# open-speech/HTK

Hardware: AMD Instinct MI355X
Metric: herest_gmm_frame_state_loglik_per_sec (higher is better)
Workload: dtype f32 (scores: bf16x3 split operands, fp32 accumulate) + f64 (alpha / beta with fp32-transcendental log-add, accumulators); 1 GPU; HERest EM iteration (pass + accumulator all-reduce + model update), 5000 tied states x 16 mix, D=39, 1250 x 500-frame utterances per GPU (BASELINE config[2]: 10k utterances sharded 8-way); states=5000, mix=16, utts_per_gpu=1250, frames=500, chunks=1, update=HERest -m 3 -v 0.01, on the device

## Files before the change

### htk_amd/capi.py

```python
from __future__ import annotations

import ctypes as C
import os

import numpy as np

from . import abi

HERE = os.path.dirname(os.path.abspath(__file__))
LIBPATH = os.path.join(HERE, "libhtk_amd.so")

LZERO = -1.0e10
LSMALL = -0.5e10
NOPRUNE = 1.0e20
UPMEANS, UPVARS, UPTRANS, UPMIXES = 1, 2, 4, 8
UPALL = 15
UPMAP = 32
UTT_OK, UTT_SKIPPED, UTT_ETEE, UTT_EALPHA = 1, 0, -7332, -7390


def _stream(s):
    return s if s is None or isinstance(s, C.c_void_p) else int(s)


# ... 275 lines not shown
    def pack_ranges(self, ranges, wire: int, dst_ptr: int, stream=None):
        self._ranges(lib().htkamd_accs_pack_ranges, ranges, wire, dst_ptr, stream)

    def unpack_ranges(self, ranges, wire: int, src_ptr: int, stream=None):
        self._ranges(lib().htkamd_accs_unpack_ranges, ranges, wire, src_ptr, stream)

    def split(self, v: np.ndarray) -> dict:
        m, L = self.model, self.lay
        GD = m.G * m.D
        return dict(vec=v, mu=v[L.mu:L.mu + GD].reshape(m.G, m.D), muOcc=v[L.muOcc:L.muOcc + m.G],
                    va=v[L.va:L.va + GD].reshape(m.G, m.D), vaOcc=v[L.vaOcc:L.vaOcc + m.G],
                    wt=v[L.wt:L.wt + m.C], wtOcc=v[L.wtOcc:L.tr], tr=v[L.tr:L.trOcc], trOcc=v[L.trOcc:L.nEgs],
                    nEgs=v[L.nEgs:L.nEgs + m.H], totalPr=v[L.totalPr], totalT=v[L.totalT], nUttDone=v[L.nUttDone],
                    nUttSkipped=v[L.nUttSkipped], nEval=v[L.nEval])


def fb_config(pruneInit=NOPRUNE, pruneInc=0.0, pruneLim=NOPRUNE, minFrwdP=10.0, uFlags=UPALL, scoreMode=0):
    return FbConfig(pruneInit, pruneInc, pruneLim, minFrwdP, uFlags, scoreMode)


class ForwardBackward(_Handle):
    _destroy = "htkamd_fb_destroy"

    def __init__(self, model: Model, debug: bool = False, force_general: bool = False, no_state_path: bool = False, stats_list: str = "auto", no_lr_path: bool = False):
        self.model = model
        self.h = C.c_void_p()
        check(lib().htkamd_fb_create(model.h, C.byref(self.h)), "fb_create")
        flags = (1 if debug else 0) | (2 if force_general else 0) | (4 if no_state_path else 0) | {"auto": 0, "tiny": 8, "off": 16}[stats_list] | (32 if no_lr_path else 0)
        if flags:
            check(lib().htkamd_fb_set_debug(self.h, flags), "fb_set_debug")
        self.nUtt = 0
        self._keep = None

    def prepare(self, dX_ptr: int, frameOff: np.ndarray, labOff: np.ndarray, labs: np.ndarray, stream=None):
        frameOff = np.ascontiguousarray(frameOff, np.int32); labOff = np.ascontiguousarray(labOff, np.int32)
        labs = np.ascontiguousarray(labs, np.int32)
        self.nUtt = len(frameOff) - 1
        self._keep = (frameOff, labOff, labs)
        b = BatchDesc(self.nUtt, dX_ptr, _p(frameOff), _p(labOff), _p(labs))
        check(lib().htkamd_fb_prepare(self.h, C.byref(b), _stream(stream)), "fb_prepare")

    def execute(self, cfg: FbConfig, accs: Accs, stream=None):
        check(lib().htkamd_fb_execute(self.h, C.byref(cfg), accs.h, _stream(stream)), "fb_execute")

    def execute_begin(self, cfg: FbConfig, accs: Accs, stream=None) -> bool:
        d = C.c_int(0)
        check(lib().htkamd_fb_execute_begin(self.h, C.byref(cfg), accs.h, _stream(stream), C.byref(d)), "fb_execute_begin")
        return bool(d.value)

    def execute_mix(self, state0: int, state1: int, stream=None):
        check(lib().htkamd_fb_execute_mix(self.h, state0, state1, _stream(stream)), "fb_execute_mix")
# ... 9 lines not shown
    def prepared_current(self) -> bool:
        return bool(lib().htkamd_fb_prepared_current(self.h))

    def frame_states(self) -> int:
        return int(lib().htkamd_fb_frame_states(self.h))

    def kernel_times(self):
        t = (C.c_double * 4)()
        check(lib().htkamd_fb_kernel_times(self.h, t), "fb_kernel_times")
        return list(t)

    def set_event_mode(self, mode: int):
        check(lib().htkamd_fb_set_event_mode(self.h, mode), "fb_set_event_mode")

    def kernel_times5(self):
        t = (C.c_double * 5)()
        check(lib().htkamd_fb_kernel_times5(self.h, t), "fb_kernel_times5")
        return list(t)

    def mix_counts(self):
        t = (C.c_longlong * 2)()
        check(lib().htkamd_fb_mix_counts(self.h, t), "fb_mix_counts")
        return int(t[0]), int(t[1])

    def score_work(self):
        t = (C.c_longlong * 3)()
        check(lib().htkamd_fb_score_work(self.h, t), "fb_score_work")
        return int(t[0]), int(t[1]), int(t[2])

    def trellis(self, u: int, want_alpha: bool = True):
        T = C.c_int(); Q = C.c_int(); mN = C.c_int()
        check(lib().htkamd_fb_get_trellis(self.h, u, None, None, None, None, None, None, None,
                                          C.byref(T), C.byref(Q), C.byref(mN), None), "fb_get_trellis")
        T, Q, mN = T.value, Q.value, mN.value
        d = dict(beta=np.empty((T, Q, mN)), alpha=np.empty((T, Q, mN)) if want_alpha else None,
                 outp=np.empty((T, Q, mN), np.float32), qLo=np.zeros(T, np.int32), qHi=np.zeros(T, np.int32),
                 aLo=np.zeros(T, np.int32), aHi=np.zeros(T, np.int32))
        check(lib().htkamd_fb_get_trellis(self.h, u, _p(d["beta"]), _p(d["alpha"]), _p(d["outp"]),
                                          _p(d["qLo"]), _p(d["qHi"]), _p(d["aLo"]), _p(d["aHi"]), None, None, None, None),
              "fb_get_trellis")
        return d


class Viterbi(_Handle):
    _destroy = "htkamd_viterbi_destroy"

# ... 1607 lines not shown
```

### htk_amd/csrc/fb.hip

```cpp
#include <hip/hip_runtime.h>
#include <cstdio>
#include <cstdlib>
#include <cstring>
#include <cmath>
#include <algorithm>
#include <vector>
#include <thread>
#include <mutex>
#include <condition_variable>
#include <functional>
#include "internal.h"
#include "hipcheck.h"
#include "kernels.h"
#include "devbuf.h"

static constexpr char fbOwner[] = "fb";
typedef DevBufT<fbOwner> DevBuf;

struct PrepPool {
   std::vector<std::thread> th;
   std::mutex mu;
   std::condition_variable cvGo, cvDone;
   std::function<void(int)> job;
   int generation = 0, pending = 0, nJobs = 0;
// ... 99 lines not shown
   Range general() const { return of(FB_LANE_PER_MODEL, 0); } int nGeneral() const { return general().n; }
   int nLr() const { return off[N] - of(FB_LEFT_TO_RIGHT, 1).first; }
   bool anyOffLr() const { return of(FB_LEFT_TO_RIGHT, 1).first > 0; }
private:
   int off[N + 1] = {};
};

struct ResLayout {
   size_t nUtt;
   size_t status() const { return sizeof(double) * nUtt; }
   size_t counter() const { return (sizeof(double) + sizeof(int)) * nUtt; }
   size_t flag() const { return counter() + sizeof(int); } size_t bytes() const { return counter() + 2 * sizeof(int); }
};

enum { UTT_NO_TEE = 1, UTT_ALL_LR = 2 };

struct htkamd_fb : BatchTables {
   htkamd_model *m = nullptr;
   int nUtt = 0;
   int debug = 0;
   int forceGeneral = 0;
   int noStatePath = 0;
   int noLrPath = 0;
   int topoVersion = 0;
   std::vector<unsigned char> uttFlags;
   UttClasses cls;
   size_t gamTotal = 0, betaWTotal = 0, alphaWTotal = 0;
   int totalFrames = 0, nCellsMax = 1, QMax = 1, TMax = 1, blockDim = 64;
   long long frameStates = 0;
   const float *dX = nullptr;
   DevBuf d_arena;
   DevBuf d_qLo, d_qHi, d_aLo, d_aHi, d_outp, d_beta, d_gam, d_alpha, d_pr;
   DevBuf d_betaW;
   DevBuf d_tmE, d_tmMaxP;
   DevBuf d_outpU;
   DevBuf d_alphaW, d_qBeam, d_aBeam, d_trPart, d_hits, d_hitCtl;
   DevBuf d_sink;
   DevBuf d_stCnt, d_stBucket;
   DevBuf d_laneRec;
   bool mixStateLast = false;
   bool mixDeferred = false;
   FbArgs *faMix = nullptr;
   const int *qBeamLast = nullptr;
   DevBuf d_transOff, d_trOccOff, d_counter;
   DevBuf d_rec, d_recSorted, d_recCtl;
   int recCapForce = 0;
   PrepPool *pool = nullptr; std::vector<PrepChunk> *chunks = nullptr;
   void *h_arena = nullptr; size_t h_arenaCap = 0;
   void *h_res = nullptr; size_t h_resCap = 0;
   hipEvent_t evRes = nullptr; bool resPending = false;
   bool f16Pass = false;
   hipEvent_t ev[6] = {}, evK[2] = {}, evCopy = nullptr;
   hipStream_t resStream = nullptr;
   bool timed = false, copyPending = false, scored = false;
   int evMode = 0, evModeLast = 0;
   ResLayout res() const { return {(size_t)nUtt}; }
};

static bool compat_revisit(const htkamd_model *m) { return (m->compat & HTKAMD_COMPAT_STREAM_REVISIT) && m->NSt > 1 && m->NSt != 3 && !m->tiedMix; }

extern "C" int htkamd_fb_create(htkamd_model *m, htkamd_fb **out)
{
// ... 16 lines not shown
   return HTKAMD_OK;
}

extern "C" void htkamd_fb_destroy(htkamd_fb *fb)
{
   if (!fb) return;
   if (fb->h_arena) (void)hipHostFree(fb->h_arena);
   if (fb->h_res) (void)hipHostFree(fb->h_res);
   delete fb->pool; delete fb->chunks; delete fb->faMix;
   for (hipEvent_t v : fb->ev) if (v) (void)hipEventDestroy(v);
   for (hipEvent_t v : {fb->evCopy, fb->evRes, fb->evK[0], fb->evK[1]}) if (v) (void)hipEventDestroy(v);
   if (fb->resStream) (void)hipStreamDestroy(fb->resStream);
   delete fb;
}

extern "C" int htkamd_fb_set_debug(htkamd_fb *fb, int on)
{
   if (!fb) { htkamd_set_error("fb_set_debug: NULL"); return HTKAMD_EINVAL; }
   fb->debug = on & 1;
   fb->forceGeneral = (on & 2) ? 1 : 0;
   fb->noStatePath = (on & 4) ? 1 : 0;
   fb->recCapForce = (on & 8) ? 128 : ((on & 16) ? -1 : 0);
   fb->noLrPath = (on & 32) ? 1 : 0;
   return HTKAMD_OK;
}

static int prep_utterance(htkamd_fb *fb, const htkamd_batch_desc *b, int u, PrepChunk &C)
{
   const htkamd_model *m = fb->m;
   std::vector<int> &evLo = C.evLo, &evHi = C.evHi;
      UttDesc &d = fb->utt[u];
      const int T = b->frameOff[u + 1] - b->frameOff[u], Q = b->labOff[u + 1] - b->labOff[u];
      const int *labs = b->labs + b->labOff[u];
      d.T = T; d.Q = Q; d.frame0 = b->frameOff[u];
      d.q0 = (int)C.mN.size(); d.cell0 = (int)C.cQ.size(); d.slot0 = (int)C.slotState.size();
      d.status = HTKAMD_UTT_OK; d.nEval = 0;
      d.outp0 = C.outp; d.beta0 = C.beta; d.gam0 = C.gam;
      unsigned char &flags = fb->uttFlags[u];
      flags = UTT_NO_TEE | UTT_ALL_LR;
      if (T <= 0 || Q <= 0) {
         for (int t = 0; t < T; t++) { fb->taperLo[d.frame0 + t] = 0; fb->taperHi[d.frame0 + t] = 0; fb->qBeamNP[d.frame0 + t] = 1; }
         d.status = HTKAMD_UTT_SKIPPED; d.nCells = d.nSlots = 0; d.thr0 = (int)C.thrCell.size(); d.nThr = 0; return HTKAMD_OK;
      }
      int nCells = 0, nSlots = 0, qt = 0, prevDm = 1;
      for (int q = 1; q <= Q; q++) {
         const int h = labs[q - 1];
// ... 404 lines not shown
}

static const int clsW[4] = {1, 2, 4, 8};

static int fb_reserve_lr(htkamd_fb *fb, const htkamd_fb_config *cfg, FbArgs &fa, bool fastLadd, hipStream_t s)
{
   const htkamd_model *m = fb->m;
   int rc;
   size_t rows = 0;
   for (int W : clsW) rows += (size_t)fb->cls.of(FB_LEFT_TO_RIGHT, W).n * htkamd_stats_lr_chunks(fb->TMax) * W;
   const size_t nfr = fb->totalFrames ? fb->totalFrames : 1;
   if ((rc = fb->d_laneRec.reserve(sizeof(LaneRec) * (fb->slotState.size() + 1))) || (rc = fb->d_sink.reserve(256))) return rc;
   fa.laneRec = (LaneRec *)fb->d_laneRec.p; fa.sink = (double *)fb->d_sink.p;
   if ((rc = fb->d_alphaW.reserve(sizeof(double) * (fb->alphaWTotal + 64))) || (rc = fb->d_qBeam.reserve(sizeof(int) * (nfr + 2))) ||
       (rc = fb->d_aBeam.reserve(sizeof(int) * (nfr + 2))) || (rc = fb->d_trPart.reserve(sizeof(double) * htkamd_stats_lr_row_doubles() * (rows + 256))) ||
       (rc = fb->d_hits.reserve(sizeof(MixHit) * (rows * htkamd_stats_lr_region_cap() + 64))) || (rc = fb->d_hitCtl.reserve(sizeof(int) * (rows + 1))))
      return rc;
   fa.alphaW = (double *)fb->d_alphaW.p; fa.qBeam = (int *)fb->d_qBeam.p; fa.aBeam = (int *)fb->d_aBeam.p; fa.trPart = (double *)fb->d_trPart.p;
   fa.hits = (MixHit *)fb->d_hits.p; fa.hitCtl = (int *)fb->d_hitCtl.p; fa.nHitRegions = (int)rows; fa.hitRegionCap = htkamd_stats_lr_region_cap();
   fa.hitSlots = (m->NSt > 1 || m->tiedMix) ? 1 : 0;
   fa.qBeamNP = fb->qBeamNP.dev;
   if (htkamd_beta_lr_is_lean(fa, fastLadd)) fa.qBeam = const_cast<int *>(fb->qBeamNP.dev);
   fb->qBeamLast = fa.qBeam;
   fb->mixStateLast = false;
   fa.fastMath = fastLadd ? 1 : 0;
   if (fb->recCapForce == 0 && !fa.hitSlots && m->maxM <= 16 && (m->D == 39 || m->D == 26 || m->D == 13) &&
       (cfg->uFlags & (HTKAMD_UPMEANS | HTKAMD_UPVARS | HTKAMD_UPMIXES))) {
      size_t cap = 64;
      while (cap < 65536 && cap * (size_t)m->S < (size_t)16 * fb->totalFrames) cap <<= 1;
      while (cap > 64 && cap * (size_t)m->S * sizeof(HitS) > ((size_t)1 << 30)) cap >>= 1;
      { const char *e = getenv("HTKAMD_ST_CAP"); if (e && atoi(e) > 0) cap = (size_t)atoi(e); }
      if ((rc = fb->d_stCnt.reserve(sizeof(int) * (3 * (size_t)m->S + 4))) || (rc = fb->d_stBucket.reserve(sizeof(HitS) * cap * (size_t)m->S))) return rc;
      fb->mixStateLast = true;
      fa.stCnt = (int *)fb->d_stCnt.p; fa.nTiedStates = m->S; fa.stBucket = (HitS *)fb->d_stBucket.p; fa.stCap = (int)cap;
      HIPCHECK(hipMemsetAsync(fa.stCnt, 0, sizeof(int) * (3 * (size_t)m->S + 4), s));
   }
   return HTKAMD_OK;
}

struct FamilyKernels { int family; int (*beta)(const FbArgs &, int, bool, hipStream_t); int (*alpha)(const FbArgs &, int, bool, hipStream_t); };
static const FamilyKernels familyKernels[] = {{FB_LANE_PER_MODEL, htkamd_launch_beta_w, htkamd_launch_alpha_w},
                                              {FB_LANE_PER_STATE, htkamd_launch_beta_s, htkamd_launch_alpha_s},
                                              {FB_LEFT_TO_RIGHT, htkamd_launch_beta_lr, htkamd_launch_alpha_lr}};

static int fb_recursions(htkamd_fb *fb, const FbArgs &fa, const LdsSizes &lds, bool fastLadd, bool noEv, hipStream_t s)
{
// ... 43 lines not shown
          (rc = fb->d_recCtl.reserve(sizeof(int) * (3 * ((size_t)m->G + 1) + 1 + (size_t)m->G / 2048 + 2))))
         return rc;
      fa.rec = (MixRec *)fb->d_rec.p; fa.recSorted = (MixRec *)fb->d_recSorted.p; fa.recCap = (int)cap; fa.G = m->G; fa.recCtl = (int *)fb->d_recCtl.p;
   }
   if (m->tiedMix || m->NSt > 1) {
      fa.stateCompOff = m->d_stateCompOff; fa.rec = nullptr;
      if (fb->nUtt > nLr && (rc = m->tiedMix ? htkamd_launch_mixstats_tm(fa, s) : htkamd_launch_mixstats_ms(fa, s))) return rc;
      if (nLr > 0 && (rc = htkamd_launch_mixhits_streams(fa, m->tiedMix != 0, s))) return rc;
      return HTKAMD_OK;
   }
   const bool dense = fb->nUtt > nLr && fa.gamTotal > 0, listed = nLr > 0;
   if ((rc = htkamd_launch_mixstats(fa, s, dense, listed, defer))) return rc;
   if (defer && listed && !dense && htkamd_mixstate_applies(fa)) {
      if (!fb->faMix) fb->faMix = new FbArgs();
      *fb->faMix = fa;
      fb->mixDeferred = true;
   }
   return HTKAMD_OK;
}

static int fb_execute_impl(htkamd_fb *fb, const htkamd_fb_config *cfg, htkamd_accs *accs, void *stream, bool defer)
{
   if (!fb || !cfg || !accs) { htkamd_set_error("fb_execute: NULL argument"); return HTKAMD_EINVAL; }
   fb->mixDeferred = false;
   if (accs->m != fb->m) { htkamd_set_error("fb_execute: accumulators belong to a different model"); return HTKAMD_EINVAL; }
   if (fb->nUtt == 0) return HTKAMD_OK;
   const htkamd_model *m = fb->m;
   hipStream_t s = (hipStream_t)stream;
   if (fb->topoVersion != m->topoVersion) {
      htkamd_set_error("fb_execute: the model's minimum durations changed since htkamd_fb_prepare (a re-estimated transition reached or left zero): prepare the batch again");
      return HTKAMD_EINVAL;
   }
   const ScoreArgs sa = fb_score_args(fb, cfg);
   if (cfg->scoreMode & ~(HTKAMD_SCORE_MFMA | HTKAMD_SCORE_FASTLADD | HTKAMD_SCORE_BF16 | HTKAMD_SCORE_F16 | HTKAMD_SCORE_SOUTP | HTKAMD_SCORE_DIAGC)) { htkamd_set_error("fb_execute: unknown score mode %d", cfg->scoreMode); return HTKAMD_EINVAL; }
   const bool fastLadd = (cfg->scoreMode & HTKAMD_SCORE_FASTLADD) != 0;
   FbArgs fa = fb_args(fb, cfg, accs);
   const LdsSizes lds = fb_lds_sizes(fa);

   int rc;
   if (fb->copyPending) HIPCHECK(hipStreamWaitEvent(s, fb->evCopy, 0));
   const bool noEv = fb->evMode == 1;
   HIPCHECK(hipEventRecord(fb->ev[0], s));
   if (m->tiedMix) {
      fa.tmE = (float *)fb->d_tmE.p; fa.tmMaxP = (float *)fb->d_tmMaxP.p; fa.tmPoolOff = m->d_tmPoolOff; fa.tmPool = m->tmPool; fa.totalFrames = fb->totalFrames;
      fa.tmTasks = fb->tasks.dev; fa.tmNTasks = (int)fb->tasks.size(); fa.tmSlotState = sa.slotState; fa.tmOut = sa.out;
      fa.compWeight = m->d_compWeight; fa.var = m->d_var;
      if ((rc = htkamd_launch_tm_score(fa, s))) return rc;
// ... 111 lines not shown
   if (!fb->timed) { htkamd_set_error("fb_kernel_times: nothing executed yet"); return HTKAMD_EINVAL; }
   HIPCHECK(hipEventSynchronize(fb->ev[5]));
   for (int i = 0; i < 5; i++) {
      float ms = 0.f;
      if (i == 0 && fb->scored) HIPCHECK(hipEventElapsedTime(&ms, fb->evK[0], fb->evK[1]));
      else if (fb->evModeLast == 1) { out[i] = -1.0; continue; }
      else HIPCHECK(hipEventElapsedTime(&ms, fb->ev[i], fb->ev[i + 1]));
      out[i] = (double)ms * 1e-3;
   }
   return HTKAMD_OK;
}

extern "C" int htkamd_fb_mix_counts(htkamd_fb *fb, long long out[2])
{
   if (!fb || !out) { htkamd_set_error("fb_mix_counts: NULL"); return HTKAMD_EINVAL; }
   out[0] = out[1] = -1;
   if (!fb->timed || !fb->mixStateLast || !fb->d_stCnt.p) return HTKAMD_OK;
   HIPCHECK(hipEventSynchronize(fb->ev[5]));
   const size_t S = (size_t)fb->m->S;
   std::vector<int> c(2 * S);
   HIPCHECK(hipMemcpy(c.data(), (int *)fb->d_stCnt.p + S + 4, sizeof(int) * 2 * S, hipMemcpyDeviceToHost));
   out[0] = out[1] = 0;
   for (size_t i = 0; i < S; i++) { out[0] += c[2 * i]; out[1] += c[2 * i + 1]; }
   return HTKAMD_OK;
}

extern "C" int htkamd_fb_kernel_times(htkamd_fb *fb, double out[4])
{
   double t[5];
   const int rc = htkamd_fb_kernel_times5(fb, t);
   if (rc) return rc;
   out[0] = t[0]; out[1] = t[1]; out[2] = (t[2] < 0.0 || t[3] < 0.0) ? -1.0 : t[2] + t[3]; out[3] = t[4];
   return HTKAMD_OK;
}

extern "C" int htkamd_fb_get_trellis(htkamd_fb *fb, int u, double *beta, double *alpha, float *outp,
                                     int *qLo, int *qHi, int *aLo, int *aHi, int *pT, int *pQ, int *pMaxN, void *stream)
{
   if (!fb || u < 0 || u >= fb->nUtt) { htkamd_set_error("fb_get_trellis: bad utterance index"); return HTKAMD_EINVAL; }
   hipStream_t s = (hipStream_t)stream;
   HIPCHECK(hipStreamSynchronize(s));
   const UttDesc &d = fb->utt[u];
   const int T = d.T, Q = d.Q, nC = d.nCells, nS = d.nSlots, maxN = fb->m->maxN;
   if (pT) *pT = T; if (pQ) *pQ = Q; if (pMaxN) *pMaxN = maxN;
   if (T <= 0 || Q <= 0) return HTKAMD_OK;
   std::vector<short> lo(T), hi(T), alo(T), ahi(T);
// ... 92 lines not shown
```

### htk_amd/csrc/fb_lr.hip

```cpp
#include <hip/hip_runtime.h>
#include <type_traits>
#include "internal.h"
#include "hipcheck.h"
#include "kernels.h"
#include "ladd.h"
#include "wavegrp.h"
#include "fb_state.h"

typedef const __attribute__((address_space(4))) int cint_lr;

#define ALPHA_S(t) (a.alphaW[ud.alphaW0 + (size_t)((t) - 1) * L + gl])
#define ALPHA_E(t, q_) (a.alphaW[ud.alphaW0 + (size_t)T * L + (size_t)((t) - 1) * ud.QP + ((q_) - 1)])

struct LrRegs {
   int q, j, N, mi;
   bool first, last;
   float aSelf, aNext, aPrev;
   float aEntry, aExit;
   float aExitPrev, aEntryNext;
};

__device__ __forceinline__ void load_lr(LrRegs &s, const FbArgs &a, const UttDesc &ud, int gl, bool valid)
{
   s.q = 0; s.j = 2; s.N = 3; s.mi = 0; s.first = false; s.last = false;
// ... 462 lines not shown
   __syncthreads();
   if (tid == 0) add_row(tb, sh[16]);
}

#include "fb_lr_lean.inc"

template <bool FAST> static void launch_beta_lr(const FbArgs &a, int W, hipStream_t s)
{
   if (W == 1) hipLaunchKernelGGL((k_beta_lr<1, FAST>), dim3(a.nList), dim3(64), 0, s, a);
   else if (W == 2) hipLaunchKernelGGL((k_beta_lr<2, FAST>), dim3(a.nList), dim3(128), 0, s, a);
   else if (W == 4) hipLaunchKernelGGL((k_beta_lr<4, FAST>), dim3(a.nList), dim3(256), 0, s, a);
   else hipLaunchKernelGGL((k_beta_lr<8, FAST>), dim3(a.nList), dim3(512), 0, s, a);
}
static void launch_alpha_lr(const FbArgs &a, int W, hipStream_t s)
{
   if (W == 1) hipLaunchKernelGGL((k_alpha_lr<1>), dim3(a.nList), dim3(64), 0, s, a);
   else if (W == 2) hipLaunchKernelGGL((k_alpha_lr<2>), dim3(a.nList), dim3(128), 0, s, a);
   else if (W == 4) hipLaunchKernelGGL((k_alpha_lr<4>), dim3(a.nList), dim3(256), 0, s, a);
   else hipLaunchKernelGGL((k_alpha_lr<8>), dim3(a.nList), dim3(512), 0, s, a);
}
template <bool DBG> static void launch_alpha_f(const FbArgs &a, int W, hipStream_t s)
{
   if (W == 1) hipLaunchKernelGGL((k_alpha_f<1, DBG>), dim3(a.nList), dim3(64), 0, s, a);
   else if (W == 2) hipLaunchKernelGGL(k_alpha_f2<DBG>, dim3(a.nList), dim3(64), 0, s, a);
   else if (W == 4) hipLaunchKernelGGL((k_alpha_f<4, DBG>), dim3(a.nList), dim3(256), 0, s, a);
   else hipLaunchKernelGGL((k_alpha_f<8, DBG>), dim3(a.nList), dim3(512), 0, s, a);
}
template <bool FAST> static void launch_stats_sp(const FbArgs &a, int W, int nChunks, hipStream_t s)
{
   if (W == 1) hipLaunchKernelGGL((k_stats_sp<1, FAST>), dim3(a.nList, nChunks), dim3(64), 0, s, a);
   else if (W == 2) hipLaunchKernelGGL((k_stats_sp<2, FAST>), dim3(a.nList, nChunks), dim3(128), 0, s, a);
   else if (W == 4) hipLaunchKernelGGL((k_stats_sp<4, FAST>), dim3(a.nList, nChunks), dim3(256), 0, s, a);
   else hipLaunchKernelGGL((k_stats_sp<8, FAST>), dim3(a.nList, nChunks), dim3(512), 0, s, a);
}

int htkamd_stats_lr_chunks(int TMax) { return (TMax + STATS_FC - 1) / STATS_FC; }
int htkamd_stats_lr_region_cap(void) { return STATS_FC * 64; }
size_t htkamd_stats_lr_row_doubles(void) { return TR_ROW; }

bool htkamd_beta_lr_is_lean(const FbArgs &a, bool fast) { return fast && a.qBeamNP && !(a.pruneInit < HTKAMD_NOPRUNE); }

int htkamd_launch_beta_lr(const FbArgs &a, int W, bool fast, hipStream_t s)
{
   if (a.nList <= 0) return HTKAMD_OK;
   if (htkamd_beta_lr_is_lean(a, fast)) {
      const dim3 grid(a.nList);
      if (W == 2) hipLaunchKernelGGL(k_beta_np2, grid, dim3(64), 0, s, a);
      else if (W == 1) hipLaunchKernelGGL((k_beta_np<1>), grid, dim3(64), 0, s, a);
      else if (W == 4) hipLaunchKernelGGL((k_beta_np<4>), grid, dim3(256), 0, s, a);
      else hipLaunchKernelGGL((k_beta_np<8>), grid, dim3(512), 0, s, a);
      HIPCHECK(hipGetLastError());
      return HTKAMD_OK;
   }
   if (fast) launch_beta_lr<true>(a, W, s); else launch_beta_lr<false>(a, W, s);
   HIPCHECK(hipGetLastError());
   return HTKAMD_OK;
}

int htkamd_launch_alpha_lr(const FbArgs &a, int W, bool fast, hipStream_t s)
{
   if (a.nList <= 0) return HTKAMD_OK;
   if (!fast) launch_alpha_lr(a, W, s);
   else if (a.alphaDbg) launch_alpha_f<true>(a, W, s);
   else launch_alpha_f<false>(a, W, s);
   HIPCHECK(hipGetLastError());
   return HTKAMD_OK;
}

int htkamd_launch_stats_lr(const FbArgs &a, int W, bool fast, hipStream_t s)
{
   if (a.nList <= 0) return HTKAMD_OK;
   const int nChunks = htkamd_stats_lr_chunks(a.TMax);
   if (fast) launch_stats_sp<true>(a, W, nChunks, s); else launch_stats_sp<false>(a, W, nChunks, s);
   const int nRows = a.nList * nChunks * W;
   hipLaunchKernelGGL(k_trans_reduce, dim3((nRows + 255) / 256), dim3(256), 0, s, a, nRows);
   HIPCHECK(hipGetLastError());
   return HTKAMD_OK;
}
```

### htk_amd/csrc/fb_lr_lean.inc

```

template <int W>
__global__ __launch_bounds__(64 * W) void k_beta_np(FbArgs a)
{
   constexpr int L = 64 * W, LP = L + 2 * SPAD;
   __shared__ double xz[2][LP];
   __shared__ double prSlot;
   const int gl = threadIdx.x;
   const int li = blockIdx.x;
   if (li >= a.nList) return;
   const int u = a.uttList[li];
   const UttDesc ud = a.utt[u];
   if (ud.status != HTKAMD_UTT_OK) {
      if (gl == 0) { a.status[u] = ud.status; a.pr[u] = LZERO; }
      return;
   }
   const int T = ud.T, Q = ud.Q, nS = ud.nSlots;
   const bool valid = gl < nS;
   LrRegs s;
   load_lr(s, a, ud, gl, valid);
   store_lane_rec(a, ud, gl, valid, s);
   for (int i = gl; i < LP; i += L) { xz[0][i] = LZERO; xz[1][i] = LZERO; }
   if (gl == 0) prSlot = LZERO;
   __syncthreads();
   const int q = s.q;
// ... 587 lines not shown
#pragma unroll
         for (int k = 0; k < BK; k++) { Rc0[k] = Rn0[k]; Rc1[k] = Rn1[k]; wc[k] = wn[k]; }
         if (b >= 1) {
            load8(Rn0, row0, b - 1); load8(Rn1, row1, b - 1);
#pragma unroll
            for (int k = 0; k < BK; k++) wn[k] = wB[BK * (b - 1) + 1 + k];
         }
#pragma unroll
         for (int k = BK - 1; k >= 0; k--) step(BK * b + k + 1, Rc0[k], Rc1[k], wc[k]);
      }
   }
   double prv = LZERO;
   if (v0 && s0.first && q0 == lo) prv = ((double)s0.aEntry + (double)o0) + b0;
   if (v1 && s1.first && q1 == lo) prv = ((double)s1.aEntry + (double)o1) + b1;
#pragma unroll
   for (int o = 32; o > 0; o >>= 1) prv = fmax(prv, __shfl_xor(prv, o));
   const int ok = prv > LSMALL;
   if (lane == 0) {
      a.pr[u] = ok ? prv : LZERO;
      a.status[u] = ok ? HTKAMD_UTT_OK : HTKAMD_UTT_SKIPPED;
   }
}

template <bool DBG>
#define ALPHA_LD(p_) __builtin_nontemporal_load((const d2s *)(p_))
#define ALPHA_LDF(p_) (*(const f4s *)(p_))
__global__ __launch_bounds__(64, LEAN2_EU) void k_alpha_f2(FbArgs a)
{
   constexpr int L = 128;
   __shared__ short flOf[L + 2];
   const int lane = threadIdx.x, g0 = 2 * lane, g1 = g0 + 1;
   const int li = blockIdx.x;
   if (li >= a.nList) return;
   const int u = a.uttList[li];
   const UttDesc ud = a.utt[u];
   if (a.status[u] != HTKAMD_UTT_OK) {
      if (lane == 0) atomicAdd(a.acc + a.lay.nUttSkipped, 1.0);
      return;
   }
   const int T = ud.T, Q = ud.Q, nS = ud.nSlots, nC = ud.nCells;
   const bool v0 = g0 < nS, v1 = g1 < nS;
   LrRegs s0, s1;
   load_lr(s0, a, ud, g0, v0); load_lr(s1, a, ud, g1, v1);
   if (v0 && s0.first) flOf[s0.q] = (short)g0;
   if (v1 && s1.first) flOf[s1.q] = (short)g1;
   if (lane == 0) { flOf[Q + 1] = (short)nS; flOf[0] = 0; }
   __syncthreads();
   const int q0 = s0.q, q1 = s1.q;
   const int cHmm0 = v0 ? a.mHmm[s0.mi] : 0, cHmm1 = v1 ? a.mHmm[s1.mi] : 0;
   const int mF0 = v0 ? g0 - (s0.j - 2) : 0x7fff, mL0 = v0 ? g0 - (s0.j - 2) + (s0.N - 3) : -1;
   const int mF1 = v1 ? g1 - (s1.j - 2) : 0x7fff, mL1 = v1 ? g1 - (s1.j - 2) + (s1.N - 3) : -1;
   const double dSelf0 = (double)s0.aSelf, dSelf1 = (double)s1.aSelf;
   const double dIn0 = (double)(s0.first ? s0.aEntry : s0.aPrev), dIn1 = (double)(s1.first ? s1.aEntry : s1.aPrev);
   const bool f0 = v0 && s0.first, f1 = v1 && s1.first;
   const double dXp0 = (f0 && q0 > 1) ? (double)s0.aExitPrev : 0.0, dXp1 = (f1 && q1 > 1) ? (double)s1.aExitPrev : 0.0;
   const double dEntry0 = (double)s0.aEntry, dEntry1 = (double)s1.aEntry;
   cint_lr *qB = (cint_lr *)(a.qBeam + ud.frame0 - 1);
   int *gaBeam = a.aBeam + ud.frame0 - 1;
   const float *row0 = a.outp + ud.outp0 + (size_t)(v0 ? g0 : 0) * T, *row1 = a.outp + ud.outp0 + (size_t)(v1 ? g1 : 0) * T;
   const double *pBeta = a.betaW + ud.betaW0 + g0;
   double *pS = a.alphaW + ud.alphaW0 + g0;
   const double pr = a.pr[u], minF = (double)a.minFrwdP;
// ... 158 lines not shown
#pragma unroll
         for (int k = 0; k < BK; k++) { Rc0[k] = Rn0[k]; Rc1[k] = Rn1[k]; Bc[k] = Bn[k]; }
         for (; ok && t <= T; t++) {
            if (t % BK == 0 && t != BK * c) load8(Rc0, Rc1, Bc, t / BK);
            const d2s bb = pickd(Bc, t % BK);
            ok = step(t, pick(Rc0, t % BK), pick(Rc1, t % BK), bb[0], bb[1], (t + 2 <= T) ? qB[t + 2] : 0, std::false_type{});
         }
      }
   }

   if (err) {
      if (lane == 0) { a.status[u] = HTKAMD_UTT_EALPHA; atomicAdd(a.acc + a.lay.nUttSkipped, 1.0); }
      return;
   }
   if (f0) atomicAdd(a.acc + a.lay.nEgs + cHmm0, 1.0);
   if (f1) atomicAdd(a.acc + a.lay.nEgs + cHmm1, 1.0);
   if (lane == 0) {
      atomicAdd(a.acc + a.lay.totalPr, pr);
      atomicAdd(a.acc + a.lay.totalT, (double)T);
      atomicAdd(a.acc + a.lay.nUttDone, 1.0);
      atomicAdd(a.acc + a.lay.nEval, (double)ud.nEval);
   }
}
```

### htk_amd/csrc/kernels.h

```cpp
#ifndef HTKAMD_KERNELS_H
#define HTKAMD_KERNELS_H
#include <hip/hip_runtime.h>
#include <vector>
#include "internal.h"

#define SCORE_TILE_FRAMES 128
#define B16_TASK_FRAMES 128
#define SCORE_TASK_SLOTS  16
#define SCORE_TASK_SLOTS_WIDE 64
#define SCORE_TASK_SLOTS_EXACT 8

struct ScoreTask {
   int frame0;
   int nFrames;
   int slot0;
   int nSlots;
   int outSlot0;
   int ldo;
   size_t outBase;
};

struct ScoreArgs {
   const ScoreTask *tasks = nullptr;
   int nTasks = 0;
// ... 134 lines not shown
   int NSt;
   const float *outpU;
   int compatRevisit;
   const int *nextSame;
   const int *dimStream;
   float *tmE;
   float *tmMaxP;
   const int *tmPoolOff;
   int tmPool, totalFrames;
   const ScoreTask *tmTasks; int tmNTasks; const int *tmSlotState; float *tmOut;
   const float *compWeight, *var;
   int tmCombine;
   const float *streamWt;
   MixHit *hits;
   int hitSlots;
   int *hitCtl;
   int nHitRegions, hitRegionCap;
   LaneRec *laneRec;
   const int *qBeamNP;
   int stBase;
   int *stCnt; int nTiedStates; HitS *stBucket; int stCap;
   int fastMath;
   double *sink;
};

int htkamd_launch_beta(const FbArgs &a, int blockDim, size_t lds, hipStream_t s);
int htkamd_launch_alpha(const FbArgs &a, int blockDim, size_t lds, hipStream_t s);
int htkamd_launch_mixstats(const FbArgs &a, hipStream_t s, bool dense, bool listed, bool deferState = false);
bool htkamd_mixstate_applies(const FbArgs &a);
int htkamd_launch_mixstate_range(const FbArgs &a, int st0, int st1, hipStream_t s);
int htkamd_launch_combine_streams(const FbArgs &a, hipStream_t s);
int htkamd_launch_mixstats_ms(const FbArgs &a, hipStream_t s);
int htkamd_launch_tm_score(const FbArgs &a, hipStream_t s);
int htkamd_launch_mixstats_tm(const FbArgs &a, hipStream_t s);
int htkamd_launch_mixhits_streams(const FbArgs &a, bool tied, hipStream_t s);
int htkamd_tm_score_block(const htkamd_model *m, const ScoreArgs &sa, int nRows, float tmBeam, hipStream_t s);
int htkamd_launch_beta_s(const FbArgs &a, int W, bool fast, hipStream_t s);
int htkamd_launch_alpha_s(const FbArgs &a, int W, bool fast, hipStream_t s);
int htkamd_launch_beta_w(const FbArgs &a, int W, bool fast, hipStream_t s);
int htkamd_launch_beta_lr(const FbArgs &a, int W, bool fast, hipStream_t s);
bool htkamd_beta_lr_is_lean(const FbArgs &a, bool fast);
int htkamd_launch_alpha_lr(const FbArgs &a, int W, bool fast, hipStream_t s);
int htkamd_launch_stats_lr(const FbArgs &a, int W, bool fast, hipStream_t s);
int htkamd_stats_lr_chunks(int TMax);
size_t htkamd_stats_lr_row_doubles(void);
int htkamd_stats_lr_region_cap(void);
int htkamd_launch_alpha_w(const FbArgs &a, int W, bool fast, hipStream_t s);

#endif
```

### include/htk_amd.h

```cpp
#ifndef HTK_AMD_H
#define HTK_AMD_H

#include <stddef.h>

#ifdef __cplusplus
extern "C" {
#endif

#define HTKAMD_OK        0
#define HTKAMD_EINVAL   (-1)
#define HTKAMD_ENODEV   (-2)
#define HTKAMD_ENOMEM   (-3)
#define HTKAMD_EHIP     (-4)
#define HTKAMD_EMODEL   (-5)
#define HTKAMD_EIO      (-6)
#define HTKAMD_ERANGE   (-7)

#define HTKAMD_LZERO    (-1.0E10)
#define HTKAMD_LSMALL   (-0.5E10)
#define HTKAMD_NOPRUNE  1.0E20

#define HTKAMD_UPMEANS  1
#define HTKAMD_UPVARS   2
#define HTKAMD_UPTRANS  4
// ... 294 lines not shown
#define HTKAMD_UTT_SKIPPED   0
#define HTKAMD_UTT_ETEE     (-7332)
#define HTKAMD_UTT_EALPHA   (-7390)

typedef struct htkamd_fb htkamd_fb;

int  htkamd_fb_create(htkamd_model *m, htkamd_fb **out);
void htkamd_fb_destroy(htkamd_fb *fb);
int  htkamd_fb_set_debug(htkamd_fb *fb, int on);
int  htkamd_fb_prepare(htkamd_fb *fb, const htkamd_batch_desc *batch, void *stream);
int  htkamd_fb_prepared_current(const htkamd_fb *fb);
int  htkamd_fb_execute(htkamd_fb *fb, const htkamd_fb_config *cfg, htkamd_accs *accs, void *stream);
int  htkamd_fb_execute_begin(htkamd_fb *fb, const htkamd_fb_config *cfg, htkamd_accs *accs, void *stream, int *deferred);
int  htkamd_fb_execute_mix(htkamd_fb *fb, int state0, int state1, void *stream);
int  htkamd_fb_results(htkamd_fb *fb, double *pr , int *status , void *stream);
int  htkamd_fb_results_begin(htkamd_fb *fb, void *stream);
long long htkamd_fb_frame_states(const htkamd_fb *fb);
int  htkamd_fb_get_trellis(htkamd_fb *fb, int utt, double *beta, double *alpha, float *outp,
                           int *qLo, int *qHi, int *aLo, int *aHi, int *T, int *Q, int *maxN, void *stream);
int  htkamd_fb_kernel_times(htkamd_fb *fb, double out[4]);
int  htkamd_fb_kernel_times5(htkamd_fb *fb, double out[5]);
int  htkamd_fb_set_event_mode(htkamd_fb *fb, int mode);
int  htkamd_fb_mix_counts(htkamd_fb *fb, long long out[2]);
int  htkamd_fb_score_work(const htkamd_fb *fb, long long out[3]);

typedef struct htkamd_viterbi htkamd_viterbi;
int  htkamd_viterbi_create(htkamd_model *m, htkamd_viterbi **out);
void htkamd_viterbi_destroy(htkamd_viterbi *v);
int  htkamd_viterbi_align(htkamd_viterbi *v, const htkamd_batch_desc *batch, float genBeam, void *stream);
int  htkamd_viterbi_align_mode(htkamd_viterbi *v, const htkamd_batch_desc *batch, float genBeam, int scoreMode, void *stream);
int  htkamd_viterbi_sizes(const htkamd_viterbi *v, size_t *nSeg , size_t *nMod );
int  htkamd_viterbi_results(htkamd_viterbi *v, int *segStart, int *segEnd, double *segScore,
                            int *modStart, int *modEnd, double *modScore,
                            double *total , int *status , void *stream);

#define HTKAMD_NODE_HMM  0
#define HTKAMD_NODE_WORD 1
#define HTKAMD_NODE_NULL 2
typedef struct {
   int nNodes, nLinks, nProns, initial, final;
   const int   *kind, *model;
   const float *pronProb;
   const int   *linkOff;
   const int   *linkDest;
   const float *linkLike;
} htkamd_net_desc;
// ... 343 lines not shown
```

Before: 29.48 billion frame-state log-lik/s.

## Add windowed 64-lane alpha kernel for two-slot-per-lane left-to-right utterances

Adds k_alpha_w64, a forward (alpha) kernel for the W==2 lean left-to-right path. A single 64-lane window slides over the 128 slots and is rebased when the beam moves past its top, instead of each lane handling two slots on every frame. Per-slot parameters are staged in LDS and score/beta rows are prefetched in blocks of eight. If the window cannot cover the beam, the kernel falls back to the original two-slot routine, which is refactored into a device function. The change adds rebase and shuffle complexity, a possible error path, and per-utterance counters exposed through a new diagnostic API.

```diff
diff --git a/htk_amd/capi.py b/htk_amd/capi.py
--- a/htk_amd/capi.py
+++ b/htk_amd/capi.py
@@ -321,11 +321,12 @@
 class ForwardBackward(_Handle):
     _destroy = "htkamd_fb_destroy"
 
-    def __init__(self, model: Model, debug: bool = False, force_general: bool = False, no_state_path: bool = False, stats_list: str = "auto", no_lr_path: bool = False):
+    def __init__(self, model: Model, debug: bool = False, force_general: bool = False, no_state_path: bool = False, stats_list: str = "auto", no_lr_path: bool = False,
+                 no_alpha_window: bool = False):
         self.model = model
         self.h = C.c_void_p()
         check(lib().htkamd_fb_create(model.h, C.byref(self.h)), "fb_create")
-        flags = (1 if debug else 0) | (2 if force_general else 0) | (4 if no_state_path else 0) | {"auto": 0, "tiny": 8, "off": 16}[stats_list] | (32 if no_lr_path else 0)
+        flags = (1 if debug else 0) | (2 if force_general else 0) | (4 if no_state_path else 0) | {"auto": 0, "tiny": 8, "off": 16}[stats_list] | (32 if no_lr_path else 0) | (64 if no_alpha_window else 0)
         if flags:
             check(lib().htkamd_fb_set_debug(self.h, flags), "fb_set_debug")
         self.nUtt = 0
@@ -381,6 +382,11 @@
         t = (C.c_longlong * 2)()
         check(lib().htkamd_fb_mix_counts(self.h, t), "fb_mix_counts")
         return int(t[0]), int(t[1])
+
+    def alpha_window_counts(self):
+        t = (C.c_longlong * 3)()
+        check(lib().htkamd_fb_alpha_window_counts(self.h, t), "fb_alpha_window_counts")
+        return int(t[0]), int(t[1]), int(t[2])
 
     def score_work(self):
         t = (C.c_longlong * 3)()
diff --git a/htk_amd/csrc/fb.hip b/htk_amd/csrc/fb.hip
--- a/htk_amd/csrc/fb.hip
+++ b/htk_amd/csrc/fb.hip
@@ -145,6 +145,7 @@
    int forceGeneral = 0;
    int noStatePath = 0;
    int noLrPath = 0;
+   int noAlphaWindow = 0;
    int topoVersion = 0;
    std::vector<unsigned char> uttFlags;
    UttClasses cls;
@@ -161,6 +162,8 @@
    DevBuf d_sink;
    DevBuf d_stCnt, d_stBucket;
    DevBuf d_laneRec;
+   DevBuf d_alphaWin;
+   bool alphaWinLast = false;
    bool mixStateLast = false;
    bool mixDeferred = false;
    FbArgs *faMix = nullptr;
@@ -223,6 +226,7 @@
    fb->noStatePath = (on & 4) ? 1 : 0;
    fb->recCapForce = (on & 8) ? 128 : ((on & 16) ? -1 : 0);
    fb->noLrPath = (on & 32) ? 1 : 0;
+   fb->noAlphaWindow = (on & 64) ? 1 : 0;
    return HTKAMD_OK;
 }
 
@@ -673,6 +677,9 @@
    fa.qBeamNP = fb->qBeamNP.dev;
    if (htkamd_beta_lr_is_lean(fa, fastLadd)) fa.qBeam = const_cast<int *>(fb->qBeamNP.dev);
    fb->qBeamLast = fa.qBeam;
+   if ((rc = fb->d_alphaWin.reserve(sizeof(int) * (2 * (size_t)fb->cls.of(FB_LEFT_TO_RIGHT, 2).n + 2)))) return rc;
+   fa.alphaWin = (int *)fb->d_alphaWin.p; fa.noAlphaWindow = fb->noAlphaWindow;
+   fb->alphaWinLast = fb->cls.of(FB_LEFT_TO_RIGHT, 2).n > 0 && htkamd_alpha_lr_is_windowed(fa, 2, fastLadd);
    fb->mixStateLast = false;
    fa.fastMath = fastLadd ? 1 : 0;
    if (fb->recCapForce == 0 && !fa.hitSlots && m->maxM <= 16 && (m->D == 39 || m->D == 26 || m->D == 13) &&
@@ -762,7 +769,7 @@
 static int fb_execute_impl(htkamd_fb *fb, const htkamd_fb_config *cfg, htkamd_accs *accs, void *stream, bool defer)
 {
    if (!fb || !cfg || !accs) { htkamd_set_error("fb_execute: NULL argument"); return HTKAMD_EINVAL; }
-   fb->mixDeferred = false;
+   fb->mixDeferred = false; fb->alphaWinLast = false;
    if (accs->m != fb->m) { htkamd_set_error("fb_execute: accumulators belong to a different model"); return HTKAMD_EINVAL; }
    if (fb->nUtt == 0) return HTKAMD_OK;
    const htkamd_model *m = fb->m;
@@ -920,6 +927,23 @@
    HIPCHECK(hipMemcpy(c.data(), (int *)fb->d_stCnt.p + S + 4, sizeof(int) * 2 * S, hipMemcpyDeviceToHost));
    out[0] = out[1] = 0;
    for (size_t i = 0; i < S; i++) { out[0] += c[2 * i]; out[1] += c[2 * i + 1]; }
+   return HTKAMD_OK;
+}
+
+extern "C" int htkamd_fb_alpha_window_counts(const htkamd_fb *fb, long long out[3])
+{
+   if (!fb || !out) { htkamd_set_error("fb_alpha_window_counts: NULL"); return HTKAMD_EINVAL; }
+   out[0] = out[1] = out[2] = -1;
+   if (!fb->timed || !fb->alphaWinLast || !fb->d_alphaWin.p) return HTKAMD_OK;
+   HIPCHECK(hipEventSynchronize(fb->ev[5]));
+   const size_t n = (size_t)fb->cls.of(FB_LEFT_TO_RIGHT, 2).n;
+   std::vector<int> c(2 * n);
+   HIPCHECK(hipMemcpy(c.data(), fb->d_alphaWin.p, sizeof(int) * 2 * n, hipMemcpyDeviceToHost));
+   out[0] = out[1] = out[2] = 0;
+   for (size_t i = 0; i < n; i++) {
+      if (c[2 * i] == 1) { out[0]++; out[1] += c[2 * i + 1]; }
+      else if (c[2 * i] == 2) out[2]++;
+   }
    return HTKAMD_OK;
 }
 
diff --git a/htk_amd/csrc/fb_lr.hip b/htk_amd/csrc/fb_lr.hip
--- a/htk_amd/csrc/fb_lr.hip
+++ b/htk_amd/csrc/fb_lr.hip
@@ -508,6 +508,7 @@
 template <bool DBG> static void launch_alpha_f(const FbArgs &a, int W, hipStream_t s)
 {
    if (W == 1) hipLaunchKernelGGL((k_alpha_f<1, DBG>), dim3(a.nList), dim3(64), 0, s, a);
+   else if (W == 2 && htkamd_alpha_lr_is_windowed(a, W, true)) hipLaunchKernelGGL(k_alpha_w64<DBG>, dim3(a.nList), dim3(64), 0, s, a);
    else if (W == 2) hipLaunchKernelGGL(k_alpha_f2<DBG>, dim3(a.nList), dim3(64), 0, s, a);
    else if (W == 4) hipLaunchKernelGGL((k_alpha_f<4, DBG>), dim3(a.nList), dim3(256), 0, s, a);
    else hipLaunchKernelGGL((k_alpha_f<8, DBG>), dim3(a.nList), dim3(512), 0, s, a);
@@ -543,6 +544,8 @@
    return HTKAMD_OK;
 }
 
+bool htkamd_alpha_lr_is_windowed(const FbArgs &a, int W, bool fast) { return fast && W == 2 && a.alphaWin && !a.noAlphaWindow; }
+
 int htkamd_launch_alpha_lr(const FbArgs &a, int W, bool fast, hipStream_t s)
 {
    if (a.nList <= 0) return HTKAMD_OK;
diff --git a/htk_amd/csrc/fb_lr_lean.inc b/htk_amd/csrc/fb_lr_lean.inc
--- a/htk_amd/csrc/fb_lr_lean.inc
+++ b/htk_amd/csrc/fb_lr_lean.inc
@@ -633,22 +633,13 @@
    }
 }
 
-template <bool DBG>
 #define ALPHA_LD(p_) __builtin_nontemporal_load((const d2s *)(p_))
 #define ALPHA_LDF(p_) (*(const f4s *)(p_))
-__global__ __launch_bounds__(64, LEAN2_EU) void k_alpha_f2(FbArgs a)
+template <bool DBG>
+__device__ __forceinline__ void alpha_f2_utt(const FbArgs &a, const int u, const UttDesc &ud, short *flOf)
 {
    constexpr int L = 128;
-   __shared__ short flOf[L + 2];
    const int lane = threadIdx.x, g0 = 2 * lane, g1 = g0 + 1;
-   const int li = blockIdx.x;
-   if (li >= a.nList) return;
-   const int u = a.uttList[li];
-   const UttDesc ud = a.utt[u];
-   if (a.status[u] != HTKAMD_UTT_OK) {
-      if (lane == 0) atomicAdd(a.acc + a.lay.nUttSkipped, 1.0);
-      return;
-   }
    const int T = ud.T, Q = ud.Q, nS = ud.nSlots, nC = ud.nCells;
    const bool v0 = g0 < nS, v1 = g1 < nS;
    LrRegs s0, s1;
@@ -853,3 +844,276 @@
       atomicAdd(a.acc + a.lay.nEval, (double)ud.nEval);
    }
 }
+
+template <bool DBG>
+__global__ __launch_bounds__(64, LEAN2_EU) void k_alpha_f2(FbArgs a)
+{
+   __shared__ short flOf[128 + 2];
+   const int li = blockIdx.x;
+   if (li >= a.nList) return;
+   const int u = a.uttList[li];
+   const UttDesc ud = a.utt[u];
+   if (a.status[u] != HTKAMD_UTT_OK) {
+      if (threadIdx.x == 0) atomicAdd(a.acc + a.lay.nUttSkipped, 1.0);
+      return;
+   }
+   alpha_f2_utt<DBG>(a, u, ud, flOf);
+}
+
+struct WinRec { float aSelf, aIn, aXp, aEntry; short q, mF, mL, first; };
+struct WinDbg { float aExit; int cell0; short j, N; };
+#define ALPHA_LD1(p_) __builtin_nontemporal_load((const double *)(p_))
+template <bool DBG>
+__global__ __launch_bounds__(64, LEAN2_EU) void k_alpha_w64(FbArgs a)
+{
+   constexpr int L = 128;
+   enum { STEP_OK = 0, STEP_ERR = 1, STEP_REBASE = 2 };
+   __shared__ short flOf[L + 2];
+   __shared__ WinRec rec[L];
+   __shared__ WinDbg dbg[DBG ? L : 1];
+   const int lane = threadIdx.x;
+   const int li = blockIdx.x;
+   if (li >= a.nList) return;
+   int *cnt = a.alphaWin + 2 * (size_t)li;
+   const int u = a.uttList[li];
+   const UttDesc ud = a.utt[u];
+   if (a.status[u] != HTKAMD_UTT_OK) {
+      if (lane == 0) { atomicAdd(a.acc + a.lay.nUttSkipped, 1.0); cnt[0] = 0; cnt[1] = 0; }
+      return;
+   }
+   const int T = ud.T, Q = ud.Q, nS = ud.nSlots, nC = ud.nCells;
+   bool fst[2]; int cHmm[2];
+#pragma unroll
+   for (int h = 0; h < 2; h++) {
+      const int gs = lane + 64 * h;
+      const bool v = gs < nS;
+      LrRegs s;
+      load_lr(s, a, ud, gs, v);
+      const bool f = v && s.first;
+      WinRec r;
+      r.aSelf = s.aSelf; r.aIn = s.first ? s.aEntry : s.aPrev; r.aXp = (f && s.q > 1) ? s.aExitPrev : 0.0f; r.aEntry = s.aEntry;
+      r.q = (short)s.q; r.mF = (short)(v ? gs - (s.j - 2) : 0x7fff); r.mL = (short)(v ? gs - (s.j - 2) + (s.N - 3) : -1); r.first = f ? 1 : 0;
+      rec[gs] = r;
+      if (f) flOf[s.q] = (short)gs;
+      fst[h] = f; cHmm[h] = v ? a.mHmm[s.mi] : 0;
+      if constexpr (DBG) { WinDbg d; d.aExit = s.aExit; d.cell0 = v ? a.mCell0[s.mi] : 0; d.j = (short)s.j; d.N = (short)s.N; dbg[gs] = d; }
+   }
+   if (lane == 0) { flOf[Q + 1] = (short)nS; flOf[0] = 0; }
+   __syncthreads();
+   cint_lr *qB = (cint_lr *)(a.qBeam + ud.frame0 - 1);
+   int *gaBeam = a.aBeam + ud.frame0 - 1;
+   const double pr = a.pr[u], minF = (double)a.minFrwdP;
+
+   int w0 = 0, g = lane, q = 0, mF = 0x7fff, mL = -1;
+   bool v = false, f = false;
+   double dSelf = LZERO, dIn = LZERO, dXp = 0.0, dEntry = LZERO;
+   unsigned long long topBit = 0;
+   const float *row = nullptr;
+   const double *pBeta = nullptr;
+   double *pS = nullptr;
+   int wCur = qB[1], wNxt = (T >= 2) ? qB[2] : wCur;
+   BeamD cur;
+   unsigned long long mX = 0;
+   auto derive = [&](const int w_) {
+      BeamD d;
+      d.lo = w_ & 0xffff; d.hi = w_ >> 16;
+      const int hh = d.hi > 0 ? d.hi : 1;
+      d.fLo = __builtin_amdgcn_readfirstlane((int)flOf[d.lo]);
+      d.fHi = __builtin_amdgcn_readfirstlane((int)flOf[hh]);
+      d.fHiEnd = __builtin_amdgcn_readfirstlane((int)flOf[hh + 1]);
+      d.fE = __builtin_amdgcn_readfirstlane((int)flOf[((hh < Q) ? hh + 1 : hh) + 1]);
+      d.inB = __ballot(q >= d.lo && q <= d.hi);
+      d.mLo = __ballot(g >= d.fLo);
+      d.mE = __ballot(g < d.fE);
+      return d;
+   };
+   auto exit_masks = [&]() {
+      const int nlo = wNxt & 0xffff, nhi = wNxt >> 16;
+      mX = __ballot(f && q > 1 && q - 1 >= cur.lo && q - 1 <= cur.hi && q >= nlo && q <= nhi);
+   };
+   auto remap = [&](const int w0_) {
+      w0 = w0_; g = w0 + lane; v = g < nS;
+      const WinRec r = rec[g];
+      q = r.q; mF = r.mF; mL = r.mL; f = r.first != 0;
+      dSelf = (double)r.aSelf; dIn = (double)r.aIn; dXp = (double)r.aXp; dEntry = (double)r.aEntry;
+      topBit = (w0 < L - 64) ? (1ull << 63) : 0ull;
+      row = a.outp + ud.outp0 + (size_t)(v ? g : 0) * T;
+      pBeta = a.betaW + ud.betaW0 + g;
+      pS = a.alphaW + ud.alphaW0 + g;
+      cur = derive(wCur);
+      exit_masks();
+   };
+   remap(0);
+
+   double aJ = LZERO, inc = LZERO;
+   double od, on = 0.0, bT, bN = LZERO;
+   int candL = -1, candH = -1, err = 0, beamV = 0, sl = 0, el = 0, nReb = 0;
+   bool fellBack = !(minF < 1.0e9) || cur.fHiEnd > 63;
+
+   auto flags = [&]() {
+      const unsigned long long k = (cur.inB & __ballot(!(pr - (aJ + bT) > minF))) | (mX & __ballot(!(pr - (inc + ((dEntry + on) + bN)) > minF)));
+      const unsigned long long l = k & cur.mLo, h = k & cur.mE;
+      candL = l ? w0 + (int)__builtin_ctzll(l) : -1;
+      candH = h ? w0 + 63 - (int)__builtin_clzll(h) : -1;
+   };
+   auto advance = [&](const int w3) {
+      if (w3 == wNxt && wNxt == wCur) return;
+      if (wNxt != wCur) { cur = derive(wNxt); wCur = wNxt; }
+      wNxt = w3;
+      exit_masks();
+   };
+   auto put_beam = [&](const int t, const int word) {
+      beamV = (lane == (t & 63)) ? word : beamV;
+      if ((t & 63) == 63 || t == T) {
+         const int tb = t & ~63;
+         if (tb + lane <= t && tb + lane >= 1) gaBeam[tb + lane] = beamV;
+      }
+   };
+   auto debug_out = [&](const int t, const double aE) {
+      if constexpr (DBG) {
+         if (a.alphaDbg) {
+            double *col = a.alphaDbg + ud.beta0 + (size_t)(t - 1) * nC;
+            auto one = [&](const int gs, const double aJs, const double aEs) {
+               if (gs >= nS) return;
+               const WinDbg d = dbg[gs];
+               double *ad = col + d.cell0;
+               ad[d.j - 1] = aJs;
+               if (d.j == 2) ad[0] = aEs;
+               if (d.j == d.N - 1) { const double aa = d.aExit; ad[d.N - 1] = (aa > LSMALL && (t == 1 || aJs > LSMALL)) ? ladd_fast(LZERO, aJs + aa) : LZERO; }
+            };
+            one(g, aJ, aE);
+            one((g + 64) & (L - 1), LZERO, LZERO);
+         }
+      }
+   };
+
+   if (!fellBack) {
+      {
+         od = (double)row[0];
+         bT = *pBeta;
+         if (T >= 2) { on = (double)row[1]; bN = pBeta[L]; }
+         const int eq = cur.hi;
+         double a1 = 0.0;
+         for (int k = 2; k <= q && k <= eq; k++) a1 += (double)(float)LZERO;
+         const bool i = v && q <= eq;
+         const double aE = i ? a1 : LZERO;
+         const double xp = aE + dEntry;
+         aJ = (i && dEntry > LSMALL) ? xp + od : LZERO;
+         sl = 0; el = cur.fHi;
+         *(i ? pS : a.sink) = xp;
+         put_beam(1, sl | (el << 16));
+         debug_out(1, aE);
+         inc = dpp_from_prev(aJ, LZERO) + dXp;
+         if (T >= 2) { flags(); advance((T >= 3) ? qB[3] : wNxt); }
+      }
+
+      auto step = [&](const int t, const float oN, const double bNn, const int qw, auto inner_) -> int {
+         constexpr bool INNER = decltype(inner_)::value;
+         const double x = ladd_fast(inc + dIn, aJ + dSelf);
+         const int l_ = candL, h_ = candH;
+         if (l_ < 0 || l_ >= cur.fHiEnd) return STEP_ERR;
+         sl = (l_ < cur.fLo) ? cur.fLo : l_;
+         if (h_ < 0 || h_ < sl) return STEP_ERR;
+         el = (h_ > cur.fHi) ? cur.fHi : h_;
+         const bool i = mL >= sl && mF <= el;
+         if (__ballot(i) & topBit) return STEP_REBASE;
+         od = on; bT = bN;
+         on = (double)oN; bN = bNn;
+         const double a1 = inc;
+         aJ = i ? x + od : LZERO;
+         *(i ? pS + (size_t)(t - 1) * L : a.sink) = x;
+         put_beam(t, sl | (el << 16));
+         debug_out(t, i ? a1 : LZERO);
+         inc = dpp_from_prev(aJ, LZERO) + dXp;
+         if (INNER || t < T) {
+            flags();
+            advance((INNER || t + 2 <= T) ? qw : wNxt);
+         }
+         return STEP_OK;
+      };
+
+      constexpr int BK = 8;
+      float Rc[BK], Rn[BK];
+      double Bc[BK], Bn[BK];
+      auto load8 = [&](float *R, double *B, const int c) {
+         const f4s a4 = ALPHA_LDF(row + BK * c), b4 = ALPHA_LDF(row + BK * c + 4);
+#pragma unroll
+         for (int k = 0; k < 4; k++) { R[k] = a4[k]; R[4 + k] = b4[k]; }
+#pragma unroll
+         for (int k = 0; k < BK; k++) B[k] = ALPHA_LD1(pBeta + (size_t)(BK * c + k) * L);
+      };
+      auto pick = [](const float *R, int k) { float x_ = R[0];
+#pragma unroll
+         for (int i = 1; i < BK; i++) x_ = (k == i) ? R[i] : x_;
+         return x_; };
+      auto pickd = [](const double *B, int k) { double x_ = B[0];
+#pragma unroll
+         for (int i = 1; i < BK; i++) x_ = (k == i) ? B[i] : x_;
+         return x_; };
+      int t = 2;
+      auto run = [&]() -> int {
+         int code = STEP_OK;
+         int c = t / BK;
+         load8(Rc, Bc, c);
+         if (BK * (c + 1) <= T) load8(Rn, Bn, c + 1);
+         for (; t <= T && t < BK * (c + 1); t++)
+            if ((code = step(t, pick(Rc, t % BK), pickd(Bc, t % BK), (t + 2 <= T) ? qB[t + 2] : 0, std::false_type{}))) return code;
+         if (t > T) return STEP_OK;
+         for (c++; BK * c + BK - 1 <= T - 2; c++) {
+#pragma unroll
+            for (int k = 0; k < BK; k++) { Rc[k] = Rn[k]; Bc[k] = Bn[k]; }
+            load8(Rn, Bn, c + 1);
+            int qw[BK];
+#pragma unroll
+            for (int k = 0; k < BK; k++) qw[k] = qB[BK * c + k + 2];
+#pragma unroll
+            for (int k = 0; k < BK; k++)
+               if ((code = step(BK * c + k, Rc[k], Bc[k], qw[k], std::true_type{}))) { t = BK * c + k; return code; }
+         }
+         t = BK * c;
+#pragma unroll
+         for (int k = 0; k < BK; k++) { Rc[k] = Rn[k]; Bc[k] = Bn[k]; }
+         for (; t <= T; t++) {
+            if (t % BK == 0 && t != BK * c) load8(Rc, Bc, t / BK);
+            if ((code = step(t, pick(Rc, t % BK), pickd(Bc, t % BK), (t + 2 <= T) ? qB[t + 2] : 0, std::false_type{}))) return code;
+         }
+         return STEP_OK;
+      };
+      while (t <= T) {
+         const int code = run();
+         if (code == STEP_OK) break;
+         if (code == STEP_ERR) { err = 1; break; }
+         const int first = __builtin_amdgcn_readfirstlane((int)rec[sl].mF);
+         const int nw = (first < L - 64) ? first : L - 64;
+         const int d = nw - w0;
+         if (d <= 0) { fellBack = true; break; }
+         const int src = lane + d;
+         const double aM = __shfl(aJ, src & 63), iM = __shfl(inc, src & 63);
+         aJ = (src < 64) ? aM : LZERO;
+         remap(nw);
+         const double ic = dpp_from_prev(aJ, LZERO) + dXp;
+         inc = (lane == 0) ? iM : ic;
+         on = (double)row[t - 1]; bN = pBeta[(size_t)(t - 1) * L];
+         nReb++;
+      }
+   }
+
+   if (fellBack) {
+      if (lane == 0) { cnt[0] = 2; cnt[1] = 0; }
+      alpha_f2_utt<DBG>(a, u, ud, flOf);
+      return;
+   }
+   if (lane == 0) { cnt[0] = err ? 0 : 1; cnt[1] = err ? 0 : nReb; }
+   if (err) {
+      if (lane == 0) { a.status[u] = HTKAMD_UTT_EALPHA; atomicAdd(a.acc + a.lay.nUttSkipped, 1.0); }
+      return;
+   }
+   if (fst[0]) atomicAdd(a.acc + a.lay.nEgs + cHmm[0], 1.0);
+   if (fst[1]) atomicAdd(a.acc + a.lay.nEgs + cHmm[1], 1.0);
+   if (lane == 0) {
+      atomicAdd(a.acc + a.lay.totalPr, pr);
+      atomicAdd(a.acc + a.lay.totalT, (double)T);
+      atomicAdd(a.acc + a.lay.nUttDone, 1.0);
+      atomicAdd(a.acc + a.lay.nEval, (double)ud.nEval);
+   }
+}
diff --git a/htk_amd/csrc/kernels.h b/htk_amd/csrc/kernels.h
--- a/htk_amd/csrc/kernels.h
+++ b/htk_amd/csrc/kernels.h
@@ -180,6 +180,8 @@
    int *stCnt; int nTiedStates; HitS *stBucket; int stCap;
    int fastMath;
    double *sink;
+   int *alphaWin;
+   int noAlphaWindow;
 };
 
 int htkamd_launch_beta(const FbArgs &a, int blockDim, size_t lds, hipStream_t s);
@@ -199,6 +201,7 @@
 int htkamd_launch_beta_lr(const FbArgs &a, int W, bool fast, hipStream_t s);
 bool htkamd_beta_lr_is_lean(const FbArgs &a, bool fast);
 int htkamd_launch_alpha_lr(const FbArgs &a, int W, bool fast, hipStream_t s);
+bool htkamd_alpha_lr_is_windowed(const FbArgs &a, int W, bool fast);
 int htkamd_launch_stats_lr(const FbArgs &a, int W, bool fast, hipStream_t s);
 int htkamd_stats_lr_chunks(int TMax);
 size_t htkamd_stats_lr_row_doubles(void);
diff --git a/include/htk_amd.h b/include/htk_amd.h
--- a/include/htk_amd.h
+++ b/include/htk_amd.h
@@ -340,6 +340,7 @@
 int  htkamd_fb_kernel_times5(htkamd_fb *fb, double out[5]);
 int  htkamd_fb_set_event_mode(htkamd_fb *fb, int mode);
 int  htkamd_fb_mix_counts(htkamd_fb *fb, long long out[2]);
+int  htkamd_fb_alpha_window_counts(const htkamd_fb *fb, long long out[3]);
 int  htkamd_fb_score_work(const htkamd_fb *fb, long long out[3]);
 
 typedef struct htkamd_viterbi htkamd_viterbi;
```

Result: no change. 29.50 billion frame-state log-lik/s (median of 5 runs) (+0.1%).
